# ChenYutongTHU/humannerf

Hardware: AMD Instinct MI355X
Metric: rendered rays/sec (128 samples/ray) at 512x512 (higher is better)
Workload: dtype f32-equivalent: split-f16 hi+lo operands, 3 f16 MFMAs, fp32 accumulate; 1 GPU; BASELINE configs[1]: 512x512 freeview frame, 262144 rays x 128 samples, eval, perturb=0, all 11 outputs of the reference Network.forward; seeded random weights of the default architecture; samples_per_ray=128, ray_chunk=32768, mlp_mode=f16x3, parallelism=frames sharded over 1 GPU(s), no collective

## Files before the change

humannerf_amd/csrc/hnrf_mlp_f16.hip:

```cpp
#include "hnrf_common.h"
#include "hnrf_sincos.h"
#include "hnrf_lds_dma.h"

namespace hnrf {

typedef float f32x16 __attribute__((ext_vector_type(16)));
typedef float f32x2 __attribute__((ext_vector_type(2)));
typedef _Float16 h16x8 __attribute__((ext_vector_type(8)));
typedef _Float16 h16x2 __attribute__((ext_vector_type(2)));

constexpr int RING = 3;
constexpr float LO_SCALE = 2048.0f;
constexpr float LO_INV = 1.0f / 2048.0f;

enum { PE16_NONE = 0, PE16_CANONICAL = 1, PE16_NONRIGID = 2 };

enum { SV_NONE = 0,
       SV_ACT = 1,
       SV_DZ = 2,
       SV_PE = 3,
       SV_ACT_H = 4,
       SV_DZ_H = 5 };
__host__ __device__ constexpr bool sv_fwd(int s) { return s == SV_ACT || s == SV_ACT_H; }
__host__ __device__ constexpr bool sv_bwd(int s) { return s == SV_DZ || s == SV_DZ_H; }
// ... 294 lines not shown
__device__ __forceinline__ void push_pair_bits(uint32_t& acc, h16x2 hh) {
    const unsigned u = __builtin_bit_cast(unsigned, hh);
    unsigned tmp;
    asm("v_pk_min_u16 %1, %2, %3\n\tv_pk_mad_u16 %0, %0, %4, %1" : "+v"(acc), "=&v"(tmp) : "v"(u), "s"(0x00010001u), "s"(0x00020002u));
}

#define HNRF_TILE_EPILOGUE_PAIR(T, I)                                                                                          \
    if constexpr (SAVE == SV_ACT) {                                                                                            \
        float x0, x1;                                                                                                          \
        epi_core<ACT, ULO>(pacc1, pacc2, I, 0u, 0, oh[2 * (T) + ((I) >> 2)], ol[2 * (T) + ((I) >> 2)], x0, x1);                \
        save_pair(*sc, bw, T, I, x0, x1);                                                                                      \
    } else if constexpr (SAVE == SV_ACT_H) {                                                                                   \
        float x0, x1;                                                                                                          \
        const h16x2 hh = epi_core<ACT, ULO>(pacc1, pacc2, I, 0u, 0, oh[2 * (T) + ((I) >> 2)], ol[2 * (T) + ((I) >> 2)], x0, x1); \
        push_pair_bits(bw[(T) >> 1], hh);                                                                                      \
        if ((I) & 1) store_frag_h(rowh, cxh, T, I, oh[2 * (T) + ((I) >> 2)]);                                                  \
    } else if constexpr (SAVE == SV_DZ) {                                                                                      \
        float x0, x1;                                                                                                          \
        epi_core<ACT_MASK_SEL, ULO>(pacc1, pacc2, I, sc->mask[(T) >> 1] >> (16 * ((T) & 1)), 0, oh[2 * (T) + ((I) >> 2)],      \
                                    ol[2 * (T) + ((I) >> 2)], x0, x1);                                                         \
        save_pair_b(*sc, T, I, x0, x1);                                                                                        \
    } else if constexpr (SAVE == SV_DZ_H) {                                                                                    \
        float x0, x1;                                                                                                          \
        const h16x2 hh = epi_core<ACT_MASK_AND, ULO>(pacc1, pacc2, I, sc->mask[(T) >> 1], 8 * ((T) & 1) + (I),                 \
                                                     oh[2 * (T) + ((I) >> 2)], ol[2 * (T) + ((I) >> 2)], x0, x1);              \
        store_pair_h(rowh, cxh, svu, T, I, hh);                                                                                \
    } else if constexpr (SAVE == SV_PE) {                                                                                      \
        sc->fout[16 * (T) + 2 * (I)] = fmaf(pacc2[2 * (I)], LO_INV, pacc1[2 * (I)]);                                           \
        sc->fout[16 * (T) + 2 * (I) + 1] = fmaf(pacc2[2 * (I) + 1], LO_INV, pacc1[2 * (I) + 1]);                               \
    } else                                                                                                                     \
        epi_pair<RELU>(pacc1, I, oh[2 * (T) + ((I) >> 2)], ol[2 * (T) + ((I) >> 2)], p.sat, p.guard);

template <int NT, int TPS, int NKA, int NKB, bool RELU, int SAVE = 0, bool PEND_IN = false, bool DEFER = false,
          int NW = 4, int NB, int NO>
__device__ __forceinline__ void layer16(Pipe& p, int nb1, int nb2, h16x8 (&bh)[NB], h16x8 (&bl)[NB],
                                        h16x8 (&oh)[NO], h16x8 (&ol)[NO], float (&last)[16], SaveCtx* sc = nullptr,
                                        f32x16* pend = nullptr) {
    static_assert(!(PEND_IN || DEFER) || SAVE == SV_NONE, "deferred epilogues exist in the inference form only");
    static_assert(!PEND_IN || NKB >= 2, "a pending tile fills the last two hidden fragments");
    static_assert(NB >= (NKB > 0 ? NKB : 1) && NO >= 2 * NT && NT % TPS == 0, "bad layer shape");
    constexpr int NK = NKA + NKB;
    constexpr int NBLK = 2 * NK;
    constexpr int NS = NT / TPS;
    constexpr int PFK = NK < 4 ? NK : 4;
    static_assert((NBLK * TPS) % NW == 0, "every wave must issue the same number of DMA pieces per slab");
    constexpr bool ULO = !sv_lifted(SAVE);
    constexpr int ACT = RELU ? ACT_RELU : ACT_NONE;
    static_assert(ULO || NT > 1, "the head layers exist in the forward kernels only");
    f32x16 pacc1 = {0.f, 0.f, 0.f, 0.f, 0.f, 0.f, 0.f, 0.f, 0.f, 0.f, 0.f, 0.f, 0.f, 0.f, 0.f, 0.f};
    f32x16 pacc2 = pacc1;
    f32x16 nbias = pacc1;
    uint32_t bw[(NT + 1) / 2];
    _Float16* const rowh = (SAVE == SV_ACT_H || SAVE == SV_DZ_H) ? sc->rowh : nullptr;
    const int cxh = (SAVE == SV_ACT_H || SAVE == SV_DZ_H) ? sc->cx : 0;
    unsigned svu = 0u;
#pragma unroll
    for (int i = 0; i < (NT + 1) / 2; ++i) bw[i] = 0u;
#pragma unroll
    for (int s = 0; s < NS; ++s) {
        const int nissue = (s + 2 < NS) ? NBLK * TPS : (s + 2 == NS ? nb1 : nb2);
        const unsigned slot2 = p.ph == 0 ? 2 : p.ph - 1;
        const int dcnt = nissue / NW;
        const char* dsrc = p.gi + p.wave * dcnt * 1024;
        const unsigned ddst = p.lds_base + p.ring_off + slot2 * p.slab_bytes + p.wave * dcnt * 1024;
        p.gi += nissue * 1024;
#pragma unroll
        for (int tt = 0; tt < TPS; ++tt) {
            const int t = s * TPS + tt;
            const unsigned lane = lane_now();
            unsigned cur = p.lds_base + p.ring_off + p.ph * p.slab_bytes + tt * (NBLK * 1024) + lane * 16;
            unsigned pe = p.lds_base + p.pe_off + p.wave * (PE_STASH / 4) + lane * 16;
            asm volatile("" : "+v"(cur), "+v"(pe));
            f32x16 acc1 = {0.f, 0.f, 0.f, 0.f, 0.f, 0.f, 0.f, 0.f, 0.f, 0.f, 0.f, 0.f, 0.f, 0.f, 0.f, 0.f};
            f32x16 acc2 = acc1;
            if (NT > 1 && sv_has_bias(SAVE)) {
                if (t == 0) {
                    const unsigned bp = p.lds_base + p.bias_off + tt * 128 + (lane >> 5) * 16;
                    const f32x4 b0 = lds_ld4f(bp), b1 = lds_ld4f(bp + 32), b2 = lds_ld4f(bp + 64), b3 = lds_ld4f(bp + 96);
                    acc1 = f32x16{b0.x, b0.y, b0.z, b0.w, b1.x, b1.y, b1.z, b1.w,
                                  b2.x, b2.y, b2.z, b2.w, b3.x, b3.y, b3.z, b3.w};
                } else {
                    acc1 = nbias;
                }
            }
            h16x8 qwh[PFK], qwl[PFK], qxh[PFK], qxl[PFK];
#pragma unroll
            for (int i = 0; i < PFK; ++i) {
                qwh[i] = lds_ld8(cur + (2 * i) * 1024);
                qwl[i] = lds_ld8(cur + (2 * i + 1) * 1024);
                if (i < NKA) {
                    qxh[i] = lds_ld8(pe + (2 * i) * 1024);
                    qxl[i] = lds_ld8(pe + (2 * i + 1) * 1024);
                }
            }
#ifdef HNRF_STAMP
            { const unsigned long long t0 = __builtin_readcyclecounter(); p.sum_b += t0 - p.t_last; p.t_last = t0; }
#endif
            __builtin_amdgcn_sched_barrier(0);
#pragma unroll
            for (int ks = 0; ks < NK; ++ks) {
                const int q = ks % PFK;
                const h16x8 wh = qwh[q], wl = qwl[q];
                h16x8 xh, xl;
                if (ks < NKA) {
                    xh = qxh[q];
                    xl = qxl[q];
                } else {
                    const int ib = ks - NKA < NB ? ks - NKA : 0;
                    xh = bh[ib];
                    xl = bl[ib];
                }
                if (ks + PFK < NK) {
                    qwl[q] = lds_ld8(cur + (2 * (ks + PFK) + 1) * 1024);
                    if (ks + PFK < NKA) qxl[q] = lds_ld8(pe + (2 * (ks + PFK) + 1) * 1024);
                    qwh[q] = lds_ld8(cur + (2 * (ks + PFK)) * 1024);
                    if (ks + PFK < NKA) qxh[q] = lds_ld8(pe + (2 * (ks + PFK)) * 1024);
                }
                acc1 = __builtin_amdgcn_mfma_f32_32x32x16_f16(wh, xh, acc1, 0, 0, 0);
                if (ULO) acc1 = __builtin_amdgcn_mfma_f32_32x32x16_f16(wh, xl, acc1, 0, 0, 0);
                else acc2 = __builtin_amdgcn_mfma_f32_32x32x16_f16(wh, xl, acc2, 0, 0, 0);
                if (ULO) acc1 = __builtin_amdgcn_mfma_f32_32x32x16_f16(wl, xh, acc1, 0, 0, 0);
                else acc2 = __builtin_amdgcn_mfma_f32_32x32x16_f16(wl, xh, acc2, 0, 0, 0);
                if (NT > 1 && sv_has_bias(SAVE) && ks == NK - 1 && t + 1 < NT) {
                    const unsigned bn = p.lds_base + p.bias_off + (tt + 1) * 128 + (lane >> 5) * 16;
                    const f32x4 b0 = lds_ld4f(bn), b1 = lds_ld4f(bn + 32), b2 = lds_ld4f(bn + 64), b3 = lds_ld4f(bn + 96);
                    nbias = f32x16{b0.x, b0.y, b0.z, b0.w, b1.x, b1.y, b1.z, b1.w,
                                   b2.x, b2.y, b2.z, b2.w, b3.x, b3.y, b3.z, b3.w};
                }
                {
                    constexpr int MAXP = (TPS * NK - 1) < 10 ? (TPS * NK - 1) : 10;
                    const int i = tt * NK + ks;
                    if (i >= 0 && i < MAXP) {
                        if (s + 2 < NS) {
                            if (i < NBLK * TPS / NW) dma_run_piece(dsrc, lane * 16, ddst, i);
                        } else if (i < dcnt) {
                            dma_run_piece(dsrc, lane * 16, ddst, i);
                        }
                    }
                }
                if (PEND_IN && t == 0) {
#pragma unroll
                    for (int i = 0; i < 8; ++i)
                        if ((i * (NK - 1)) / 8 == ks) {
                            epi_pair<true>(*pend, i, bh[NKB - 2 + (i >> 2)], bl[NKB - 2 + (i >> 2)], p.sat, p.guard);
                            asm volatile("" : "+v"(bh[NKB - 2 + (i >> 2)]), "+v"(bl[NKB - 2 + (i >> 2)]));
                        }
                }
                if (t > 0) {
#pragma unroll
                    for (int i = 0; i < 8; ++i)
                        if ((i * NK) / 8 == ks) {
                            HNRF_TILE_EPILOGUE_PAIR(t - 1, i)
                            if constexpr (SAVE != SV_PE)
                                asm volatile("" : "+v"(oh[2 * (t - 1) + (i >> 2)]), "+v"(ol[2 * (t - 1) + (i >> 2)]));
                        }
                }
                __builtin_amdgcn_sched_group_barrier(0x008, 1, 0);
                __builtin_amdgcn_sched_group_barrier(0x002, 6, 0);
                __builtin_amdgcn_sched_group_barrier(0x008, 1, 0);
                __builtin_amdgcn_sched_group_barrier(0x100, 2, 0);
                __builtin_amdgcn_sched_group_barrier(0x002, 5, 0);
                __builtin_amdgcn_sched_group_barrier(0x008, 1, 0);
                __builtin_amdgcn_sched_group_barrier(0x002, 8, 0);
                __builtin_amdgcn_sched_barrier(0);
            }
#ifdef HNRF_STAMP
            { const unsigned long long t1 = __builtin_readcyclecounter(); p.sum_k += t1 - p.t_last; p.t_last = t1; }
#endif
            pacc1 = acc1;
            pacc2 = acc2;
        }
        const int n_st = (sv_fwd(SAVE) || sv_bwd(SAVE)) ? 4 * (s == 0 ? TPS - 1 : TPS) : 0;
        tile_sync(nissue / NW + n_st);
        p.ph = p.ph == RING - 1 ? 0 : p.ph + 1;
        p.bias_off += TPS * 128;
    }
    if (NT == 1) {
#pragma unroll
        for (int r = 0; r < 16; ++r) last[r] = pacc1[r];
    } else if (DEFER) {
        *pend = pacc1;
    } else {
#pragma unroll
        for (int i = 0; i < 8; ++i) {
            HNRF_TILE_EPILOGUE_PAIR(NT - 1, i)
        }
        if constexpr (sv_fwd(SAVE)) {
#pragma unroll
            for (int i = 0; i < (NT + 1) / 2; ++i) sc->bits[i] = bw[i];
        }
    }
}

#undef HNRF_TILE_EPILOGUE_PAIR

template <int NT, int TPS, int NKA, int NKB, bool RELU, int NB, int NO>
__device__ __forceinline__ void layer16x2(Pipe& p, unsigned stash_per_wave, int nb1, int nb2,
                                          const h16x8 (&bh)[2][NB], const h16x8 (&bl)[2][NB], h16x8 (&oh)[2][NO],
                                          h16x8 (&ol)[2][NO], float (&last)[2][16]) {
    static_assert(NB >= (NKB > 0 ? NKB : 1) && NO >= 2 * NT && NT % TPS == 0, "bad layer shape");
    constexpr int NK = NKA + NKB;
    constexpr int NBLK = 2 * NK;
    constexpr int NS = NT / TPS;
    constexpr int PFK = NK < 4 ? NK : 4;
    static_assert((NBLK * TPS) % 4 == 0, "every wave must issue the same number of DMA pieces per slab");
    const f32x16 zero = {0.f, 0.f, 0.f, 0.f, 0.f, 0.f, 0.f, 0.f, 0.f, 0.f, 0.f, 0.f, 0.f, 0.f, 0.f, 0.f};
    f32x16 pacc[2] = {zero, zero};
#pragma unroll
    for (int s = 0; s < NS; ++s) {
        const int nissue = (s + 2 < NS) ? NBLK * TPS : (s + 2 == NS ? nb1 : nb2);
        const unsigned slot2 = p.ph == 0 ? 2 : p.ph - 1;
        const int dcnt = nissue / 4;
        const char* dsrc = p.gi + p.wave * dcnt * 1024;
        const unsigned ddst = p.lds_base + p.ring_off + slot2 * p.slab_bytes + p.wave * dcnt * 1024;
        p.gi += nissue * 1024;
#pragma unroll
        for (int tt = 0; tt < TPS; ++tt) {
            const int t = s * TPS + tt;
            const unsigned lane = lane_now();
            unsigned cur = p.lds_base + p.ring_off + p.ph * p.slab_bytes + tt * (NBLK * 1024) + lane * 16;
            unsigned pe = p.lds_base + p.pe_off + p.wave * stash_per_wave + lane * 16;
            asm volatile("" : "+v"(cur), "+v"(pe));
            f32x16 acc[2] = {zero, zero};
            if (NT > 1) {
                const unsigned bp = p.lds_base + p.bias_off + tt * 128 + (lane >> 5) * 16;
                const f32x4 b0 = lds_ld4f(bp), b1 = lds_ld4f(bp + 32), b2 = lds_ld4f(bp + 64), b3 = lds_ld4f(bp + 96);
                acc[0] = f32x16{b0.x, b0.y, b0.z, b0.w, b1.x, b1.y, b1.z, b1.w,
                                 b2.x, b2.y, b2.z, b2.w, b3.x, b3.y, b3.z, b3.w};
                acc[1] = acc[0];
            }
            h16x8 qwh[PFK], qwl[PFK], qxh[2][PFK], qxl[2][PFK];
#pragma unroll
            for (int i = 0; i < PFK; ++i) {
                qwh[i] = lds_ld8(cur + (2 * i) * 1024);
                qwl[i] = lds_ld8(cur + (2 * i + 1) * 1024);
                if (i < NKA) {
#pragma unroll
                    for (int g = 0; g < 2; ++g) {
                        qxh[g][i] = lds_ld8(pe + g * (stash_per_wave / 2) + (2 * i) * 1024);
                        qxl[g][i] = lds_ld8(pe + g * (stash_per_wave / 2) + (2 * i + 1) * 1024);
                    }
                }
            }
            __builtin_amdgcn_sched_barrier(0);
#pragma unroll
            for (int ks = 0; ks < NK; ++ks) {
                const int q = ks % PFK;
                const h16x8 wh = qwh[q], wl = qwl[q];
                h16x8 xh[2], xl[2];
#pragma unroll
                for (int g = 0; g < 2; ++g) {
                    if (ks < NKA) {
                        xh[g] = qxh[g][q];
                        xl[g] = qxl[g][q];
                    } else {
                        const int ib = ks - NKA < NB ? ks - NKA : 0;
                        xh[g] = bh[g][ib];
                        xl[g] = bl[g][ib];
                    }
                }
                if (ks + PFK < NK) {
                    qwl[q] = lds_ld8(cur + (2 * (ks + PFK) + 1) * 1024);
                    if (ks + PFK < NKA) {
#pragma unroll
                        for (int g = 1; g >= 0; --g) qxl[g][q] = lds_ld8(pe + g * (stash_per_wave / 2) + (2 * (ks + PFK) + 1) * 1024);
                    }
                    qwh[q] = lds_ld8(cur + (2 * (ks + PFK)) * 1024);
                    if (ks + PFK < NKA) {
#pragma unroll
                        for (int g = 1; g >= 0; --g) qxh[g][q] = lds_ld8(pe + g * (stash_per_wave / 2) + (2 * (ks + PFK)) * 1024);
                    }
                }
#pragma unroll
                for (int g = 0; g < 2; ++g) {
                    acc[g] = __builtin_amdgcn_mfma_f32_32x32x16_f16(wh, xh[g], acc[g], 0, 0, 0);
                    acc[g] = __builtin_amdgcn_mfma_f32_32x32x16_f16(wh, xl[g], acc[g], 0, 0, 0);
                    acc[g] = __builtin_amdgcn_mfma_f32_32x32x16_f16(wl, xh[g], acc[g], 0, 0, 0);
                }
                {
                    constexpr int MAXP = (TPS * NK - 1) < 10 ? (TPS * NK - 1) : 10;
                    const int i = tt * NK + ks;
                    if (i >= 0 && i < MAXP) {
                        if (s + 2 < NS) {
                            if (i < NBLK * TPS / 4) dma_run_piece(dsrc, lane * 16, ddst, i);
                        } else if (i < dcnt) {
                            dma_run_piece(dsrc, lane * 16, ddst, i);
                        }
                    }
                }
                if (t > 0) {
#pragma unroll
                    for (int j = 0; j < 16; ++j)
                        if ((j * NK) / 16 == ks) {
                            const int g = j >> 3, i = j & 7;
                            epi_pair<RELU>(pacc[g], i, oh[g][2 * (t - 1) + (i >> 2)], ol[g][2 * (t - 1) + (i >> 2)], p.sat, p.guard);
                            asm volatile("" : "+v"(oh[g][2 * (t - 1) + (i >> 2)]), "+v"(ol[g][2 * (t - 1) + (i >> 2)]));
                        }
                }
                __builtin_amdgcn_sched_group_barrier(0x008, 1, 0);
                __builtin_amdgcn_sched_group_barrier(0x002, 6, 0);
                __builtin_amdgcn_sched_group_barrier(0x008, 1, 0);
                __builtin_amdgcn_sched_group_barrier(0x100, 2, 0);
                __builtin_amdgcn_sched_group_barrier(0x002, 5, 0);
                __builtin_amdgcn_sched_group_barrier(0x008, 1, 0);
                __builtin_amdgcn_sched_group_barrier(0x100, 2, 0);
                __builtin_amdgcn_sched_group_barrier(0x002, 5, 0);
                __builtin_amdgcn_sched_group_barrier(0x008, 1, 0);
                __builtin_amdgcn_sched_group_barrier(0x002, 6, 0);
                __builtin_amdgcn_sched_group_barrier(0x008, 1, 0);
                __builtin_amdgcn_sched_group_barrier(0x100, 2, 0);
                __builtin_amdgcn_sched_group_barrier(0x002, 5, 0);
                __builtin_amdgcn_sched_group_barrier(0x008, 1, 0);
                __builtin_amdgcn_sched_group_barrier(0x002, 8, 0);
                __builtin_amdgcn_sched_barrier(0);
            }
#pragma unroll
            for (int g = 0; g < 2; ++g) pacc[g] = acc[g];
        }
        tile_sync(nissue / 4);
        p.ph = p.ph == RING - 1 ? 0 : p.ph + 1;
        p.bias_off += TPS * 128;
    }
#pragma unroll
    for (int g = 0; g < 2; ++g) {
        if (NT == 1) {
#pragma unroll
            for (int r = 0; r < 16; ++r) last[g][r] = pacc[g][r];
        } else {
#pragma unroll
            for (int i = 0; i < 8; ++i)
                epi_pair<RELU>(pacc[g], i, oh[g][2 * (NT - 1) + (i >> 2)], ol[g][2 * (NT - 1) + (i >> 2)], p.sat, p.guard);
        }
    }
}

__device__ __forceinline__ Pipe pipe_start(const char* packed, int64_t bias_img_off, int bias_bytes, int slab_bytes,
                                           int nb0, int nb1, char* smem, int stash_bytes = PE_STASH, int nw = 4) {
    Pipe p;
    p.wave = __builtin_amdgcn_readfirstlane(threadIdx.x >> 6);
    p.lds_base = __builtin_amdgcn_readfirstlane((unsigned)(size_t)(lds_char*)smem);
    p.pe_off = bias_bytes;
    p.ring_off = bias_bytes + stash_bytes;
    p.slab_bytes = slab_bytes;
    p.ph = 0;
    p.bias_off = 0;
    p.sat = 0ull;
    p.guard = false;
#ifdef HNRF_STAMP
    p.t_last = __builtin_readcyclecounter();
    p.sum_k = p.sum_b = 0;
#endif
    slab_issue(packed + bias_img_off, p.lds_base, bias_bytes / 1024, p.wave, nw);
    slab_issue(packed, p.lds_base + p.ring_off, nb0, p.wave, nw);
    slab_issue(packed + nb0 * 1024, p.lds_base + p.ring_off + slab_bytes, nb1, p.wave, nw);
    p.gi = packed + (nb0 + nb1) * 1024;
    return p;
}

template <bool ULO = false>
__device__ __forceinline__ void stash_pe(const Pipe& p, int ks, const float (&v)[8]) {
    h16x8 hi, lo;
    split8<ULO>(v, hi, lo);
    const unsigned pe = p.lds_base + p.pe_off + p.wave * (PE_STASH / 4) + lane_now() * 16;
    lds_st8(pe + (2 * ks) * 1024, hi);
    lds_st8(pe + (2 * ks + 1) * 1024, lo);
}

// ... 75 lines not shown
    layer16<1, 1, 0, 16, false, 0, DF, false>(p, 0, 0, hA_h, hA_l, dh, dl, last, nullptr, &pend);
    const float* ob = reinterpret_cast<const float*>(packed + CNL16_BIAS + CNL16_BIAS_LDS);
    if constexpr (HEADS) {
        if (slot < P) {
#pragma unroll
            for (int q = 0; q < 4; ++q) {
                const int g = 2 * q + h;
                if (g < n_heads) {
                    const float hs = h ? ob[32 + 2 * q + 1] : ob[32 + 2 * q];
                    const float* bg = ob + 4 * g;
                    raw[(int64_t)g * plane + sample] = make_float4(fmaf(last[4 * q], hs, bg[0]), fmaf(last[4 * q + 1], hs, bg[1]),
                                                                   fmaf(last[4 * q + 2], hs, bg[2]), fmaf(last[4 * q + 3], hs, bg[3]));
                }
            }
        }
    } else {
        const float hs = ob[8];
        if (h == 0 && slot < P)
            raw[sample] = make_float4(fmaf(last[0], hs, ob[0]), fmaf(last[1], hs, ob[1]), fmaf(last[2], hs, ob[2]), fmaf(last[3], hs, ob[3]));
    }
    if constexpr (SAVE == SV_NONE && GUARD) raise_f16_range(packed, CNL16_STATUS, p.sat);
#ifdef HNRF_STAMP
    if (threadIdx.x == 0 && blockIdx.x < 4096) {
        const unsigned long long te = __builtin_readcyclecounter();
        unsigned long long* dbg = (unsigned long long*)(const_cast<char*>(packed) + CNL16_BYTES);
        dbg[blockIdx.x * 4 + 0] = p.sum_k; dbg[blockIdx.x * 4 + 1] = p.sum_b + (te - p.t_last);
    }
#endif
}

constexpr int NR16W8_SLAB = 24 * 1024;
constexpr int NR16W8_STASH = 64 * 1024;

template <int SAVE, int NW = 4>
__global__ __launch_bounds__(64 * NW) void nonrigid_f16x3_kernel(const float* __restrict__ x_skel,
                                                             const float* __restrict__ hann_w,
                                                             const char* __restrict__ packed, int64_t P,
                                                             float* __restrict__ xyz, float* __restrict__ offsets,
                                                             const int* __restrict__ idx,
                                                             const int* __restrict__ count,
                                                             float* __restrict__ pe_out, float* __restrict__ acts,
                                                             uint32_t* __restrict__ relu_bits) {
    extern __shared__ __attribute__((aligned(16))) char smem[];
    if (idx != nullptr) {
        P = *count;
        if ((int64_t)blockIdx.x * (32 * NW) >= P) return;
    }
    static_assert(NW == 4 || NW == 8, "waves per workgroup");
    constexpr bool W8 = NW == 8;
    Pipe p = W8 ? pipe_start(packed, NR16_BIAS, NR16_BIAS_LDS, NR16W8_SLAB, 2 * NR16_NB_L0, 2 * NR16_NB_L0, smem, NR16W8_STASH, 8)
                : pipe_start(packed, NR16_BIAS, NR16_BIAS_LDS, NR16_SLAB, 4 * NR16_NB_L0, 2 * NR16_NB_MID, smem);
    const int lane = threadIdx.x & 63, h = lane >> 5;
    const int64_t slot = ((int64_t)blockIdx.x * NW + p.wave) * 32 + (lane & 31);
    const int64_t sclamp = slot < P ? slot : P - 1;
    const int64_t sidx = idx ? (int64_t)idx[sclamp] : sclamp;
    const int64_t sample = slot < P ? sidx : P;

    const float x[3] = {x_skel[sidx * 3 + 0], x_skel[sidx * 3 + 1], x_skel[sidx * 3 + 2]};
    float pev[32];
    pe_sincos_shared<6>(x, h, pev);
#pragma unroll
    for (int a = 0; a < 18; ++a) pev[a] *= hann_w[a / 3];
#pragma unroll
    for (int a = 18; a < 32; ++a) pev[a] = 0.f;
#pragma unroll
    for (int ks = 0; ks < 4; ++ks) {
        const float v[8] = {pev[8 * ks], pev[8 * ks + 1], pev[8 * ks + 2], pev[8 * ks + 3],
                            pev[8 * ks + 4], pev[8 * ks + 5], pev[8 * ks + 6], pev[8 * ks + 7]};
        stash_pe<true>(p, ks, v);
    }
    SaveCtx sc;
    if constexpr (SAVE) {
        sc.row = acts + sidx * 128 + 4 * h;
        sc.rowh = reinterpret_cast<_Float16*>(acts) + (slot >> 5) * (128 * 32) + h * 128;
        sc.cx = (lane & 31) ^ (4 * h);
        sc.bits = relu_bits + sidx * 4 + 2 * h;
        if constexpr (SAVE == SV_ACT_H) {
            _Float16* ph = reinterpret_cast<_Float16*>(pe_out) + sidx * 64;
#pragma unroll
            for (int a = 0; a < 18; ++a) ph[pe_col16(PE16_NONRIGID, a, h)] = (_Float16)pev[a];
#pragma unroll
            for (int a = 18; a < 32; ++a) ph[36 + 2 * (a - 18) + h] = (_Float16)0.f;
        } else {
#pragma unroll
            for (int a = 0; a < 18; ++a) pe_out[sidx * 36 + pe_col16(PE16_NONRIGID, a, h)] = pev[a];
        }
    }
    const int64_t act_stride = P * 128, bit_stride = P * 4;
    const int64_t acth_stride = (int64_t)gridDim.x * (32 * NW) * 128;
    tile_sync(0);

    h16x8 hA_h[8], hA_l[8], hB_h[8], hB_l[8];
    float last[16];
    h16x8 dh[2], dl[2];
    if constexpr (W8) {
        constexpr int MID = NR16_NB_MID, L4B = NR16_NB_L4;
#define HNRF_NEXT_LAYER if constexpr (SAVE) { sc.row += act_stride; sc.rowh += acth_stride; sc.bits += bit_stride; }
        layer16<4, 2, 4, 0, true, SAVE, false, false, 8>(p, MID, MID, hB_h, hB_l, hA_h, hA_l, last, &sc);
        HNRF_NEXT_LAYER
        layer16<4, 1, 0, 8, true, SAVE, false, false, 8>(p, MID, MID, hA_h, hA_l, hB_h, hB_l, last, &sc);
        HNRF_NEXT_LAYER
        layer16<4, 1, 0, 8, true, SAVE, false, false, 8>(p, MID, MID, hB_h, hB_l, hA_h, hA_l, last, &sc);
        HNRF_NEXT_LAYER
        layer16<4, 1, 0, 8, true, SAVE, false, false, 8>(p, L4B, L4B, hA_h, hA_l, hB_h, hB_l, last, &sc);
        HNRF_NEXT_LAYER
        layer16<4, 1, 4, 8, true, SAVE, false, false, 8>(p, MID, MID, hB_h, hB_l, hA_h, hA_l, last, &sc);
        HNRF_NEXT_LAYER
        layer16<4, 1, 0, 8, true, SAVE, false, false, 8>(p, MID, 0, hA_h, hA_l, hB_h, hB_l, last, &sc);
#undef HNRF_NEXT_LAYER
        layer16<1, 1, 0, 8, false, 0, false, false, 8>(p, 0, 0, hB_h, hB_l, dh, dl, last);
    } else {
    layer16<4, 4, 4, 0, true, SAVE>(p, 0 , 2 * NR16_NB_MID, hB_h, hB_l, hA_h, hA_l, last, &sc);
    if constexpr (SAVE) { sc.row += act_stride; sc.rowh += acth_stride; sc.bits += bit_stride; }
    layer16<4, 2, 0, 8, true, SAVE>(p, 2 * NR16_NB_MID, 2 * NR16_NB_MID, hA_h, hA_l, hB_h, hB_l, last, &sc);
    if constexpr (SAVE) { sc.row += act_stride; sc.rowh += acth_stride; sc.bits += bit_stride; }
    layer16<4, 2, 0, 8, true, SAVE>(p, 2 * NR16_NB_MID, 2 * NR16_NB_MID, hB_h, hB_l, hA_h, hA_l, last, &sc);
    if constexpr (SAVE) { sc.row += act_stride; sc.rowh += acth_stride; sc.bits += bit_stride; }
    layer16<4, 2, 0, 8, true, SAVE>(p, NR16_NB_L4, NR16_NB_L4, hA_h, hA_l, hB_h, hB_l, last, &sc);
    if constexpr (SAVE) { sc.row += act_stride; sc.rowh += acth_stride; sc.bits += bit_stride; }
    layer16<4, 1, 4, 8, true, SAVE>(p, 2 * NR16_NB_MID, 2 * NR16_NB_MID, hB_h, hB_l, hA_h, hA_l, last, &sc);
    if constexpr (SAVE) { sc.row += act_stride; sc.rowh += acth_stride; sc.bits += bit_stride; }
    layer16<4, 2, 0, 8, true, SAVE>(p, NR16_NB_MID, 0, hA_h, hA_l, hB_h, hB_l, last, &sc);
    layer16<1, 1, 0, 8, false, 0>(p, 0, 0, hB_h, hB_l, dh, dl, last);
    }
    const float* ob = reinterpret_cast<const float*>(packed + NR16_BIAS + NR16_BIAS_LDS);
    const float hs = ob[8];
    if (h == 0 && slot < P) {
        const float o0 = fmaf(last[0], hs, ob[0]), o1 = fmaf(last[1], hs, ob[1]), o2 = fmaf(last[2], hs, ob[2]);
        xyz[sample * 3 + 0] = x[0] + o0;
        xyz[sample * 3 + 1] = x[1] + o1;
        xyz[sample * 3 + 2] = x[2] + o2;
        if (offsets) {
            offsets[sample * 3 + 0] = o0;
            offsets[sample * 3 + 1] = o1;
            offsets[sample * 3 + 2] = o2;
        }
    }
}

constexpr int NR16X2_SLAB = 24 * 1024;
constexpr int NR16X2_STASH = 64 * 1024;

template <bool GUARD>
__global__ __launch_bounds__(256) void nonrigid_f16x3_x2_kernel(const float* __restrict__ x_skel,
                                                                const float* __restrict__ hann_w,
                                                                const char* __restrict__ packed, int64_t P,
                                                                float* __restrict__ xyz, float* __restrict__ offsets,
                                                                const int* __restrict__ idx,
                                                                const int* __restrict__ count) {
    extern __shared__ __attribute__((aligned(16))) char smem[];
    if (idx != nullptr) {
        P = *count;
        if ((int64_t)blockIdx.x * 256 >= P) return;
    }
    Pipe p = pipe_start(packed, NR16_BIAS, NR16_BIAS_LDS, NR16X2_SLAB, 2 * NR16_NB_L0, 2 * NR16_NB_L0, smem,
                        NR16X2_STASH);
    p.guard = GUARD;
    constexpr unsigned SPW = NR16X2_STASH / 4;
    const int lane = threadIdx.x & 63, h = lane >> 5;
    int64_t sidx[2];
    bool live[2];
    float x[2][3];
#pragma unroll
    for (int g = 0; g < 2; ++g) {
        const int64_t slot = ((int64_t)blockIdx.x * 4 + p.wave) * 64 + g * 32 + (lane & 31);
        const int64_t sclamp = slot < P ? slot : P - 1;
        sidx[g] = idx ? (int64_t)idx[sclamp] : sclamp;
        live[g] = slot < P;
#pragma unroll
        for (int a = 0; a < 3; ++a) x[g][a] = x_skel[sidx[g] * 3 + a];
    }
#pragma unroll
    for (int g = 0; g < 2; ++g) {
        float pev[32];
        pe_sincos_shared<6>(x[g], h, pev);
#pragma unroll
        for (int a = 0; a < 18; ++a) pev[a] *= hann_w[a / 3];
#pragma unroll
        for (int a = 18; a < 32; ++a) pev[a] = 0.f;
        const unsigned pe = p.lds_base + p.pe_off + p.wave * SPW + g * (SPW / 2) + lane_now() * 16;
#pragma unroll
        for (int ks = 0; ks < 4; ++ks) {
            const float v[8] = {pev[8 * ks], pev[8 * ks + 1], pev[8 * ks + 2], pev[8 * ks + 3],
                                pev[8 * ks + 4], pev[8 * ks + 5], pev[8 * ks + 6], pev[8 * ks + 7]};
            h16x8 hi, lo;
            split8<true>(v, hi, lo);
            lds_st8(pe + (2 * ks) * 1024, hi);
            lds_st8(pe + (2 * ks + 1) * 1024, lo);
        }
    }
    tile_sync(0);

    h16x8 hA_h[2][8], hA_l[2][8], hB_h[2][8], hB_l[2][8];
    float last[2][16];
    constexpr int MID = NR16_NB_MID, L4B = NR16_NB_L4;
    layer16x2<4, 2, 4, 0, true>(p, SPW, MID, MID, hB_h, hB_l, hA_h, hA_l, last);
    layer16x2<4, 1, 0, 8, true>(p, SPW, MID, MID, hA_h, hA_l, hB_h, hB_l, last);
    layer16x2<4, 1, 0, 8, true>(p, SPW, MID, MID, hB_h, hB_l, hA_h, hA_l, last);
    layer16x2<4, 1, 0, 8, true>(p, SPW, L4B, L4B, hA_h, hA_l, hB_h, hB_l, last);
    layer16x2<4, 1, 4, 8, true>(p, SPW, MID, MID, hB_h, hB_l, hA_h, hA_l, last);
    layer16x2<4, 1, 0, 8, true>(p, SPW, MID, 0, hA_h, hA_l, hB_h, hB_l, last);
    h16x8 dh[2][2], dl[2][2];
    layer16x2<1, 1, 0, 8, false>(p, SPW, 0, 0, hB_h, hB_l, dh, dl, last);
    const float* ob = reinterpret_cast<const float*>(packed + NR16_BIAS + NR16_BIAS_LDS);
    const float hs = ob[8];
#pragma unroll
    for (int g = 0; g < 2; ++g) {
        if (h == 0 && live[g]) {
            const float o0 = fmaf(last[g][0], hs, ob[0]), o1 = fmaf(last[g][1], hs, ob[1]), o2 = fmaf(last[g][2], hs, ob[2]);
            xyz[sidx[g] * 3 + 0] = x[g][0] + o0;
            xyz[sidx[g] * 3 + 1] = x[g][1] + o1;
            xyz[sidx[g] * 3 + 2] = x[g][2] + o2;
            if (offsets) {
                offsets[sidx[g] * 3 + 0] = o0;
                offsets[sidx[g] * 3 + 1] = o1;
                offsets[sidx[g] * 3 + 2] = o2;
            }
        }
    }
    if constexpr (GUARD) raise_f16_range(packed, NR16_STATUS, p.sat);
}

struct PackBwd16 {
    const float* W;
    int n_out, n_in;
    int NT, NK;
    int row_kind;
    int col0;
    int head;
    int64_t off;
    const float* amax;
};

struct LayerSet {
    const float* w[9];
    int n[9];
};
__global__ __launch_bounds__(256) void layer_amax_kernel(LayerSet ls, float* __restrict__ out) {
    __shared__ float red[256];
    const float* W = ls.w[blockIdx.x];
    const int n = ls.n[blockIdx.x];
    float m = 0.f;
    for (int e = blockIdx.y * 256 + threadIdx.x; e < n; e += 256 * gridDim.y) m = fmaxf(m, fabsf(W[e]));
    red[threadIdx.x] = m;
    __syncthreads();
    for (int st = 128; st >= 1; st >>= 1) {
        if ((int)threadIdx.x < st) red[threadIdx.x] = fmaxf(red[threadIdx.x], red[threadIdx.x + st]);
        __syncthreads();
    }
    if (threadIdx.x == 0) atomicMax(reinterpret_cast<unsigned int*>(out) + blockIdx.x, __float_as_uint(red[0]));
}

struct PackBwdSet16 {
// ... 378 lines not shown
    return launch_lds<canonical_f16x3_kernel<SV_NONE, false, true>>(what, grid, dim3(256), lds, st, xyz, (const char*)packed, P,
                                                                    (float4*)raw, idx, count, nullptr, nullptr, nullptr,
                                                                    n_heads);
}

int canonical16_fwd_train(const float* xyz, const void* packed, int64_t P, float* raw, float* pe_out, float* acts,
                          uint32_t* relu_bits, int half, hipStream_t st) {
    constexpr int lds = CNL16_BIAS_LDS + PE_STASH + RING * CNL16_SLAB;
    const dim3 grid((unsigned)((P + 127) / 128));
    const char* what = "hnrf_canonical_fwd_train (f16x3)";
    if (half)
        return launch_lds<canonical_f16x3_kernel<SV_ACT_H>>(what, grid, dim3(256), lds, st, xyz, (const char*)packed, P,
                                                            (float4*)raw, nullptr, nullptr, pe_out, acts, relu_bits, 1);
    return launch_lds<canonical_f16x3_kernel<SV_ACT>>(what, grid, dim3(256), lds, st, xyz, (const char*)packed, P, (float4*)raw,
                                                      nullptr, nullptr, pe_out, acts, relu_bits, 1);
}

int canonical16_heads_fwd_train(const float* xyz, const void* packed, int64_t P, int n_heads, float* raw, float* pe_out,
                                float* acts, uint32_t* relu_bits, int half, hipStream_t st) {
    constexpr int lds = CNL16_BIAS_LDS + PE_STASH + RING * CNL16_SLAB;
    const dim3 grid((unsigned)((P + 127) / 128));
    const char* what = "hnrf_canonical_heads_fwd_train (f16x3)";
    if (half)
        return launch_lds<canonical_f16x3_kernel<SV_ACT_H, false, true>>(what, grid, dim3(256), lds, st, xyz, (const char*)packed,
                                                                         P, (float4*)raw, nullptr, nullptr, pe_out, acts,
                                                                         relu_bits, n_heads);
    return launch_lds<canonical_f16x3_kernel<SV_ACT, false, true>>(what, grid, dim3(256), lds, st, xyz, (const char*)packed, P,
                                                                   (float4*)raw, nullptr, nullptr, pe_out, acts, relu_bits,
                                                                   n_heads);
}

int nonrigid16_fwd(const float* x_skel, const float* hann_w, const void* packed, int64_t P, float* xyz,
                   float* offsets, const int* idx, const int* count, bool guard, hipStream_t st) {
    constexpr int lds2 = NR16_BIAS_LDS + NR16X2_STASH + RING * NR16X2_SLAB;
    const dim3 grid((unsigned)((P + 255) / 256));
    const char* what = "hnrf_nonrigid_fwd (f16x3)";
    if (guard)
        return launch_lds<nonrigid_f16x3_x2_kernel<true>>(what, grid, dim3(256), lds2, st, x_skel, hann_w, (const char*)packed, P,
                                                          xyz, offsets, idx, count);
    return launch_lds<nonrigid_f16x3_x2_kernel<false>>(what, grid, dim3(256), lds2, st, x_skel, hann_w, (const char*)packed, P,
                                                       xyz, offsets, idx, count);
}

int nonrigid16_fwd_train(const float* x_skel, const float* hann_w, const void* packed, int64_t P, float* xyz,
                         float* offsets, float* pe_out, float* acts, uint32_t* relu_bits, int half, hipStream_t st) {
    constexpr int lds = NR16_BIAS_LDS + PE_STASH + RING * NR16_SLAB;
    const dim3 grid((unsigned)((P + 127) / 128));
    const char* what = "hnrf_nonrigid_fwd_train (f16x3)";
    if (half && P % 256 == 0) {
        constexpr int lds8 = NR16_BIAS_LDS + NR16W8_STASH + RING * NR16W8_SLAB;
        return launch_lds<nonrigid_f16x3_kernel<SV_ACT_H, 8>>(what, dim3((unsigned)(P / 256)), dim3(512), lds8, st, x_skel, hann_w,
                                                              (const char*)packed, P, xyz, offsets, nullptr, nullptr, pe_out,
                                                              acts, relu_bits);
    }
    if (half)
        return launch_lds<nonrigid_f16x3_kernel<SV_ACT_H>>(what, grid, dim3(256), lds, st, x_skel, hann_w, (const char*)packed, P,
                                                           xyz, offsets, nullptr, nullptr, pe_out, acts, relu_bits);
    return launch_lds<nonrigid_f16x3_kernel<SV_ACT>>(what, grid, dim3(256), lds, st, x_skel, hann_w, (const char*)packed, P, xyz,
                                                     offsets, nullptr, nullptr, pe_out, acts, relu_bits);
}

size_t canonical16_bwd_bytes() { return (size_t)CB16_BYTES + 256; }

static int launch_layer_amax(const float* const* w, const int* n, int count, float* out, hipStream_t st) {
    LayerSet ls;
    for (int i = 0; i < 9; ++i) { ls.w[i] = i < count ? w[i] : nullptr; ls.n[i] = i < count ? n[i] : 0; }
    if (hipMemsetAsync(out, 0, 256, st) != hipSuccess) {
        set_error("hnrf pack (layer maxima): memset failed");
        return HNRF_E_LAUNCH;
    }
    hipLaunchKernelGGL(layer_amax_kernel, dim3(count, 16), dim3(256), 0, st, ls, out);
    return check_launch("hnrf pack (layer maxima)");
}

// ... 110 lines not shown
```

Baseline: 4.968 million rays/s.

## Route nonrigid inference through 8-wave kernel with deferred epilogues and mid-slab sync

Removes the dedicated two-group nonrigid inference kernel. Inference now runs through the 8-wave nonrigid kernel (512 threads, one 32-row tile per wave) with deferred epilogues. A new MIDSYNC mode moves the ring barrier to the middle of each slab's MFMA loop and issues the next slab's DMA pieces after it, so the barrier is hidden behind compute instead of sitting at the slab's end. The trade is more waves per block and a different barrier placement, which may change register pressure and occupancy compared with the old register-blocked two-group design.

New measurement: 4.989 million rays/s (median of 6 runs). Within noise of the previous version (+0.4%).

```diff
diff --git a/humannerf_amd/csrc/hnrf_mlp_f16.hip b/humannerf_amd/csrc/hnrf_mlp_f16.hip
--- a/humannerf_amd/csrc/hnrf_mlp_f16.hip
+++ b/humannerf_amd/csrc/hnrf_mlp_f16.hip
@@ -350,7 +350,7 @@
         epi_pair<RELU>(pacc1, I, oh[2 * (T) + ((I) >> 2)], ol[2 * (T) + ((I) >> 2)], p.sat, p.guard);
 
 template <int NT, int TPS, int NKA, int NKB, bool RELU, int SAVE = 0, bool PEND_IN = false, bool DEFER = false,
-          int NW = 4, int NB, int NO>
+          int NW = 4, bool MIDSYNC = false, int NB, int NO>
 __device__ __forceinline__ void layer16(Pipe& p, int nb1, int nb2, h16x8 (&bh)[NB], h16x8 (&bl)[NB],
                                         h16x8 (&oh)[NO], h16x8 (&ol)[NO], float (&last)[16], SaveCtx* sc = nullptr,
                                         f32x16* pend = nullptr) {
@@ -365,6 +365,9 @@
     constexpr bool ULO = !sv_lifted(SAVE);
     constexpr int ACT = RELU ? ACT_RELU : ACT_NONE;
     static_assert(ULO || NT > 1, "the head layers exist in the forward kernels only");
+    static_assert(!MIDSYNC || SAVE == SV_NONE, "the activation stores of the training forms are counted at the slab's end");
+    constexpr int MS = TPS * NK / 2;
+    static_assert(!MIDSYNC || 24 / NW <= TPS * NK - MS, "a slab's pieces (at most 24 blocks) are issued behind the meeting");
     f32x16 pacc1 = {0.f, 0.f, 0.f, 0.f, 0.f, 0.f, 0.f, 0.f, 0.f, 0.f, 0.f, 0.f, 0.f, 0.f, 0.f, 0.f};
     f32x16 pacc2 = pacc1;
     f32x16 nbias = pacc1;
@@ -417,6 +420,10 @@
             __builtin_amdgcn_sched_barrier(0);
 #pragma unroll
             for (int ks = 0; ks < NK; ++ks) {
+                if (MIDSYNC && tt * NK + ks == MS) {
+                    tile_sync(0);
+                    __builtin_amdgcn_sched_barrier(0);
+                }
                 const int q = ks % PFK;
                 const h16x8 wh = qwh[q], wl = qwl[q];
                 h16x8 xh, xl;
@@ -447,7 +454,7 @@
                 }
                 {
                     constexpr int MAXP = (TPS * NK - 1) < 10 ? (TPS * NK - 1) : 10;
-                    const int i = tt * NK + ks;
+                    const int i = tt * NK + ks - (MIDSYNC ? MS : 0);
                     if (i >= 0 && i < MAXP) {
                         if (s + 2 < NS) {
                             if (i < NBLK * TPS / NW) dma_run_piece(dsrc, lane * 16, ddst, i);
@@ -489,7 +496,7 @@
             pacc2 = acc2;
         }
         const int n_st = (sv_fwd(SAVE) || sv_bwd(SAVE)) ? 4 * (s == 0 ? TPS - 1 : TPS) : 0;
-        tile_sync(nissue / NW + n_st);
+        if constexpr (!MIDSYNC) tile_sync(nissue / NW + n_st);
         p.ph = p.ph == RING - 1 ? 0 : p.ph + 1;
         p.bias_off += TPS * 128;
     }
@@ -511,146 +518,6 @@
 }
 
 #undef HNRF_TILE_EPILOGUE_PAIR
-
-template <int NT, int TPS, int NKA, int NKB, bool RELU, int NB, int NO>
-__device__ __forceinline__ void layer16x2(Pipe& p, unsigned stash_per_wave, int nb1, int nb2,
-                                          const h16x8 (&bh)[2][NB], const h16x8 (&bl)[2][NB], h16x8 (&oh)[2][NO],
-                                          h16x8 (&ol)[2][NO], float (&last)[2][16]) {
-    static_assert(NB >= (NKB > 0 ? NKB : 1) && NO >= 2 * NT && NT % TPS == 0, "bad layer shape");
-    constexpr int NK = NKA + NKB;
-    constexpr int NBLK = 2 * NK;
-    constexpr int NS = NT / TPS;
-    constexpr int PFK = NK < 4 ? NK : 4;
-    static_assert((NBLK * TPS) % 4 == 0, "every wave must issue the same number of DMA pieces per slab");
-    const f32x16 zero = {0.f, 0.f, 0.f, 0.f, 0.f, 0.f, 0.f, 0.f, 0.f, 0.f, 0.f, 0.f, 0.f, 0.f, 0.f, 0.f};
-    f32x16 pacc[2] = {zero, zero};
-#pragma unroll
-    for (int s = 0; s < NS; ++s) {
-        const int nissue = (s + 2 < NS) ? NBLK * TPS : (s + 2 == NS ? nb1 : nb2);
-        const unsigned slot2 = p.ph == 0 ? 2 : p.ph - 1;
-        const int dcnt = nissue / 4;
-        const char* dsrc = p.gi + p.wave * dcnt * 1024;
-        const unsigned ddst = p.lds_base + p.ring_off + slot2 * p.slab_bytes + p.wave * dcnt * 1024;
-        p.gi += nissue * 1024;
-#pragma unroll
-        for (int tt = 0; tt < TPS; ++tt) {
-            const int t = s * TPS + tt;
-            const unsigned lane = lane_now();
-            unsigned cur = p.lds_base + p.ring_off + p.ph * p.slab_bytes + tt * (NBLK * 1024) + lane * 16;
-            unsigned pe = p.lds_base + p.pe_off + p.wave * stash_per_wave + lane * 16;
-            asm volatile("" : "+v"(cur), "+v"(pe));
-            f32x16 acc[2] = {zero, zero};
-            if (NT > 1) {
-                const unsigned bp = p.lds_base + p.bias_off + tt * 128 + (lane >> 5) * 16;
-                const f32x4 b0 = lds_ld4f(bp), b1 = lds_ld4f(bp + 32), b2 = lds_ld4f(bp + 64), b3 = lds_ld4f(bp + 96);
-                acc[0] = f32x16{b0.x, b0.y, b0.z, b0.w, b1.x, b1.y, b1.z, b1.w,
-                                 b2.x, b2.y, b2.z, b2.w, b3.x, b3.y, b3.z, b3.w};
-                acc[1] = acc[0];
-            }
-            h16x8 qwh[PFK], qwl[PFK], qxh[2][PFK], qxl[2][PFK];
-#pragma unroll
-            for (int i = 0; i < PFK; ++i) {
-                qwh[i] = lds_ld8(cur + (2 * i) * 1024);
-                qwl[i] = lds_ld8(cur + (2 * i + 1) * 1024);
-                if (i < NKA) {
-#pragma unroll
-                    for (int g = 0; g < 2; ++g) {
-                        qxh[g][i] = lds_ld8(pe + g * (stash_per_wave / 2) + (2 * i) * 1024);
-                        qxl[g][i] = lds_ld8(pe + g * (stash_per_wave / 2) + (2 * i + 1) * 1024);
-                    }
-                }
-            }
-            __builtin_amdgcn_sched_barrier(0);
-#pragma unroll
-            for (int ks = 0; ks < NK; ++ks) {
-                const int q = ks % PFK;
-                const h16x8 wh = qwh[q], wl = qwl[q];
-                h16x8 xh[2], xl[2];
-#pragma unroll
-                for (int g = 0; g < 2; ++g) {
-                    if (ks < NKA) {
-                        xh[g] = qxh[g][q];
-                        xl[g] = qxl[g][q];
-                    } else {
-                        const int ib = ks - NKA < NB ? ks - NKA : 0;
-                        xh[g] = bh[g][ib];
-                        xl[g] = bl[g][ib];
-                    }
-                }
-                if (ks + PFK < NK) {
-                    qwl[q] = lds_ld8(cur + (2 * (ks + PFK) + 1) * 1024);
-                    if (ks + PFK < NKA) {
-#pragma unroll
-                        for (int g = 1; g >= 0; --g) qxl[g][q] = lds_ld8(pe + g * (stash_per_wave / 2) + (2 * (ks + PFK) + 1) * 1024);
-                    }
-                    qwh[q] = lds_ld8(cur + (2 * (ks + PFK)) * 1024);
-                    if (ks + PFK < NKA) {
-#pragma unroll
-                        for (int g = 1; g >= 0; --g) qxh[g][q] = lds_ld8(pe + g * (stash_per_wave / 2) + (2 * (ks + PFK)) * 1024);
-                    }
-                }
-#pragma unroll
-                for (int g = 0; g < 2; ++g) {
-                    acc[g] = __builtin_amdgcn_mfma_f32_32x32x16_f16(wh, xh[g], acc[g], 0, 0, 0);
-                    acc[g] = __builtin_amdgcn_mfma_f32_32x32x16_f16(wh, xl[g], acc[g], 0, 0, 0);
-                    acc[g] = __builtin_amdgcn_mfma_f32_32x32x16_f16(wl, xh[g], acc[g], 0, 0, 0);
-                }
-                {
-                    constexpr int MAXP = (TPS * NK - 1) < 10 ? (TPS * NK - 1) : 10;
-                    const int i = tt * NK + ks;
-                    if (i >= 0 && i < MAXP) {
-                        if (s + 2 < NS) {
-                            if (i < NBLK * TPS / 4) dma_run_piece(dsrc, lane * 16, ddst, i);
-                        } else if (i < dcnt) {
-                            dma_run_piece(dsrc, lane * 16, ddst, i);
-                        }
-                    }
-                }
-                if (t > 0) {
-#pragma unroll
-                    for (int j = 0; j < 16; ++j)
-                        if ((j * NK) / 16 == ks) {
-                            const int g = j >> 3, i = j & 7;
-                            epi_pair<RELU>(pacc[g], i, oh[g][2 * (t - 1) + (i >> 2)], ol[g][2 * (t - 1) + (i >> 2)], p.sat, p.guard);
-                            asm volatile("" : "+v"(oh[g][2 * (t - 1) + (i >> 2)]), "+v"(ol[g][2 * (t - 1) + (i >> 2)]));
-                        }
-                }
-                __builtin_amdgcn_sched_group_barrier(0x008, 1, 0);
-                __builtin_amdgcn_sched_group_barrier(0x002, 6, 0);
-                __builtin_amdgcn_sched_group_barrier(0x008, 1, 0);
-                __builtin_amdgcn_sched_group_barrier(0x100, 2, 0);
-                __builtin_amdgcn_sched_group_barrier(0x002, 5, 0);
-                __builtin_amdgcn_sched_group_barrier(0x008, 1, 0);
-                __builtin_amdgcn_sched_group_barrier(0x100, 2, 0);
-                __builtin_amdgcn_sched_group_barrier(0x002, 5, 0);
-                __builtin_amdgcn_sched_group_barrier(0x008, 1, 0);
-                __builtin_amdgcn_sched_group_barrier(0x002, 6, 0);
-                __builtin_amdgcn_sched_group_barrier(0x008, 1, 0);
-                __builtin_amdgcn_sched_group_barrier(0x100, 2, 0);
-                __builtin_amdgcn_sched_group_barrier(0x002, 5, 0);
-                __builtin_amdgcn_sched_group_barrier(0x008, 1, 0);
-                __builtin_amdgcn_sched_group_barrier(0x002, 8, 0);
-                __builtin_amdgcn_sched_barrier(0);
-            }
-#pragma unroll
-            for (int g = 0; g < 2; ++g) pacc[g] = acc[g];
-        }
-        tile_sync(nissue / 4);
-        p.ph = p.ph == RING - 1 ? 0 : p.ph + 1;
-        p.bias_off += TPS * 128;
-    }
-#pragma unroll
-    for (int g = 0; g < 2; ++g) {
-        if (NT == 1) {
-#pragma unroll
-            for (int r = 0; r < 16; ++r) last[g][r] = pacc[g][r];
-        } else {
-#pragma unroll
-            for (int i = 0; i < 8; ++i)
-                epi_pair<RELU>(pacc[g], i, oh[g][2 * (NT - 1) + (i >> 2)], ol[g][2 * (NT - 1) + (i >> 2)], p.sat, p.guard);
-        }
-    }
-}
 
 __device__ __forceinline__ Pipe pipe_start(const char* packed, int64_t bias_img_off, int bias_bytes, int slab_bytes,
                                            int nb0, int nb1, char* smem, int stash_bytes = PE_STASH, int nw = 4) {
@@ -792,7 +659,7 @@
 constexpr int NR16W8_SLAB = 24 * 1024;
 constexpr int NR16W8_STASH = 64 * 1024;
 
-template <int SAVE, int NW = 4>
+template <int SAVE, int NW = 4, bool GUARD = false>
 __global__ __launch_bounds__(64 * NW) void nonrigid_f16x3_kernel(const float* __restrict__ x_skel,
                                                              const float* __restrict__ hann_w,
                                                              const char* __restrict__ packed, int64_t P,
@@ -810,6 +677,7 @@
     constexpr bool W8 = NW == 8;
     Pipe p = W8 ? pipe_start(packed, NR16_BIAS, NR16_BIAS_LDS, NR16W8_SLAB, 2 * NR16_NB_L0, 2 * NR16_NB_L0, smem, NR16W8_STASH, 8)
                 : pipe_start(packed, NR16_BIAS, NR16_BIAS_LDS, NR16_SLAB, 4 * NR16_NB_L0, 2 * NR16_NB_MID, smem);
+    p.guard = GUARD && SAVE == SV_NONE;
     const int lane = threadIdx.x & 63, h = lane >> 5;
     const int64_t slot = ((int64_t)blockIdx.x * NW + p.wave) * 32 + (lane & 31);
     const int64_t sclamp = slot < P ? slot : P - 1;
@@ -849,26 +717,31 @@
     const int64_t act_stride = P * 128, bit_stride = P * 4;
     const int64_t acth_stride = (int64_t)gridDim.x * (32 * NW) * 128;
     tile_sync(0);
+#ifdef HNRF_STAMP
+    const unsigned long long t_pro = __builtin_readcyclecounter() - p.t_last;
+#endif
 
     h16x8 hA_h[8], hA_l[8], hB_h[8], hB_l[8];
     float last[16];
     h16x8 dh[2], dl[2];
     if constexpr (W8) {
         constexpr int MID = NR16_NB_MID, L4B = NR16_NB_L4;
+        constexpr bool INF = SAVE == SV_NONE;
+        f32x16 pend;
 #define HNRF_NEXT_LAYER if constexpr (SAVE) { sc.row += act_stride; sc.rowh += acth_stride; sc.bits += bit_stride; }
-        layer16<4, 2, 4, 0, true, SAVE, false, false, 8>(p, MID, MID, hB_h, hB_l, hA_h, hA_l, last, &sc);
+        layer16<4, 2, 4, 0, true, SAVE, false, INF, 8, INF>(p, MID, MID, hB_h, hB_l, hA_h, hA_l, last, &sc, &pend);
         HNRF_NEXT_LAYER
-        layer16<4, 1, 0, 8, true, SAVE, false, false, 8>(p, MID, MID, hA_h, hA_l, hB_h, hB_l, last, &sc);
+        layer16<4, 1, 0, 8, true, SAVE, INF, INF, 8, INF>(p, MID, MID, hA_h, hA_l, hB_h, hB_l, last, &sc, &pend);
         HNRF_NEXT_LAYER
-        layer16<4, 1, 0, 8, true, SAVE, false, false, 8>(p, MID, MID, hB_h, hB_l, hA_h, hA_l, last, &sc);
+        layer16<4, 1, 0, 8, true, SAVE, INF, INF, 8, INF>(p, MID, MID, hB_h, hB_l, hA_h, hA_l, last, &sc, &pend);
         HNRF_NEXT_LAYER
-        layer16<4, 1, 0, 8, true, SAVE, false, false, 8>(p, L4B, L4B, hA_h, hA_l, hB_h, hB_l, last, &sc);
+        layer16<4, 1, 0, 8, true, SAVE, INF, INF, 8, INF>(p, L4B, L4B, hA_h, hA_l, hB_h, hB_l, last, &sc, &pend);
         HNRF_NEXT_LAYER
-        layer16<4, 1, 4, 8, true, SAVE, false, false, 8>(p, MID, MID, hB_h, hB_l, hA_h, hA_l, last, &sc);
+        layer16<4, 1, 4, 8, true, SAVE, INF, INF, 8, INF>(p, MID, MID, hB_h, hB_l, hA_h, hA_l, last, &sc, &pend);
         HNRF_NEXT_LAYER
-        layer16<4, 1, 0, 8, true, SAVE, false, false, 8>(p, MID, 0, hA_h, hA_l, hB_h, hB_l, last, &sc);
+        layer16<4, 1, 0, 8, true, SAVE, INF, INF, 8, INF>(p, MID, 0, hA_h, hA_l, hB_h, hB_l, last, &sc, &pend);
 #undef HNRF_NEXT_LAYER
-        layer16<1, 1, 0, 8, false, 0, false, false, 8>(p, 0, 0, hB_h, hB_l, dh, dl, last);
+        layer16<1, 1, 0, 8, false, 0, INF, false, 8, INF>(p, 0, 0, hB_h, hB_l, dh, dl, last, nullptr, &pend);
     } else {
     layer16<4, 4, 4, 0, true, SAVE>(p, 0 , 2 * NR16_NB_MID, hB_h, hB_l, hA_h, hA_l, last, &sc);
     if constexpr (SAVE) { sc.row += act_stride; sc.rowh += acth_stride; sc.bits += bit_stride; }
@@ -896,89 +769,14 @@
             offsets[sample * 3 + 2] = o2;
         }
     }
-}
-
-constexpr int NR16X2_SLAB = 24 * 1024;
-constexpr int NR16X2_STASH = 64 * 1024;
-
-template <bool GUARD>
-__global__ __launch_bounds__(256) void nonrigid_f16x3_x2_kernel(const float* __restrict__ x_skel,
-                                                                const float* __restrict__ hann_w,
-                                                                const char* __restrict__ packed, int64_t P,
-                                                                float* __restrict__ xyz, float* __restrict__ offsets,
-                                                                const int* __restrict__ idx,
-                                                                const int* __restrict__ count) {
-    extern __shared__ __attribute__((aligned(16))) char smem[];
-    if (idx != nullptr) {
-        P = *count;
-        if ((int64_t)blockIdx.x * 256 >= P) return;
-    }
-    Pipe p = pipe_start(packed, NR16_BIAS, NR16_BIAS_LDS, NR16X2_SLAB, 2 * NR16_NB_L0, 2 * NR16_NB_L0, smem,
-                        NR16X2_STASH);
-    p.guard = GUARD;
-    constexpr unsigned SPW = NR16X2_STASH / 4;
-    const int lane = threadIdx.x & 63, h = lane >> 5;
-    int64_t sidx[2];
-    bool live[2];
-    float x[2][3];
-#pragma unroll
-    for (int g = 0; g < 2; ++g) {
-        const int64_t slot = ((int64_t)blockIdx.x * 4 + p.wave) * 64 + g * 32 + (lane & 31);
-        const int64_t sclamp = slot < P ? slot : P - 1;
-        sidx[g] = idx ? (int64_t)idx[sclamp] : sclamp;
-        live[g] = slot < P;
-#pragma unroll
-        for (int a = 0; a < 3; ++a) x[g][a] = x_skel[sidx[g] * 3 + a];
-    }
-#pragma unroll
-    for (int g = 0; g < 2; ++g) {
-        float pev[32];
-        pe_sincos_shared<6>(x[g], h, pev);
-#pragma unroll
-        for (int a = 0; a < 18; ++a) pev[a] *= hann_w[a / 3];
-#pragma unroll
-        for (int a = 18; a < 32; ++a) pev[a] = 0.f;
-        const unsigned pe = p.lds_base + p.pe_off + p.wave * SPW + g * (SPW / 2) + lane_now() * 16;
-#pragma unroll
-        for (int ks = 0; ks < 4; ++ks) {
-            const float v[8] = {pev[8 * ks], pev[8 * ks + 1], pev[8 * ks + 2], pev[8 * ks + 3],
-                                pev[8 * ks + 4], pev[8 * ks + 5], pev[8 * ks + 6], pev[8 * ks + 7]};
-            h16x8 hi, lo;
-            split8<true>(v, hi, lo);
-            lds_st8(pe + (2 * ks) * 1024, hi);
-            lds_st8(pe + (2 * ks + 1) * 1024, lo);
-        }
-    }
-    tile_sync(0);
-
-    h16x8 hA_h[2][8], hA_l[2][8], hB_h[2][8], hB_l[2][8];
-    float last[2][16];
-    constexpr int MID = NR16_NB_MID, L4B = NR16_NB_L4;
-    layer16x2<4, 2, 4, 0, true>(p, SPW, MID, MID, hB_h, hB_l, hA_h, hA_l, last);
-    layer16x2<4, 1, 0, 8, true>(p, SPW, MID, MID, hA_h, hA_l, hB_h, hB_l, last);
-    layer16x2<4, 1, 0, 8, true>(p, SPW, MID, MID, hB_h, hB_l, hA_h, hA_l, last);
-    layer16x2<4, 1, 0, 8, true>(p, SPW, L4B, L4B, hA_h, hA_l, hB_h, hB_l, last);
-    layer16x2<4, 1, 4, 8, true>(p, SPW, MID, MID, hB_h, hB_l, hA_h, hA_l, last);
-    layer16x2<4, 1, 0, 8, true>(p, SPW, MID, 0, hA_h, hA_l, hB_h, hB_l, last);
-    h16x8 dh[2][2], dl[2][2];
-    layer16x2<1, 1, 0, 8, false>(p, SPW, 0, 0, hB_h, hB_l, dh, dl, last);
-    const float* ob = reinterpret_cast<const float*>(packed + NR16_BIAS + NR16_BIAS_LDS);
-    const float hs = ob[8];
-#pragma unroll
-    for (int g = 0; g < 2; ++g) {
-        if (h == 0 && live[g]) {
-            const float o0 = fmaf(last[g][0], hs, ob[0]), o1 = fmaf(last[g][1], hs, ob[1]), o2 = fmaf(last[g][2], hs, ob[2]);
-            xyz[sidx[g] * 3 + 0] = x[g][0] + o0;
-            xyz[sidx[g] * 3 + 1] = x[g][1] + o1;
-            xyz[sidx[g] * 3 + 2] = x[g][2] + o2;
-            if (offsets) {
-                offsets[sidx[g] * 3 + 0] = o0;
-                offsets[sidx[g] * 3 + 1] = o1;
-                offsets[sidx[g] * 3 + 2] = o2;
-            }
-        }
-    }
-    if constexpr (GUARD) raise_f16_range(packed, NR16_STATUS, p.sat);
+    if constexpr (SAVE == SV_NONE && GUARD) raise_f16_range(packed, NR16_STATUS, p.sat);
+#ifdef HNRF_STAMP
+    if ((threadIdx.x & 63) == 0 && (p.wave & 3) == 0 && blockIdx.x < 4096) {
+        const unsigned long long te = __builtin_readcyclecounter();
+        unsigned long long* dbg = (unsigned long long*)(const_cast<char*>(packed) + NR16_BYTES) + (blockIdx.x * 2 + (p.wave >> 2)) * 4;
+        dbg[0] = p.sum_k; dbg[1] = p.sum_b + (te - p.t_last); dbg[2] = t_pro; dbg[3] = te - p.t_last;
+    }
+#endif
 }
 
 struct PackBwd16 {
@@ -1423,14 +1221,15 @@
 
 int nonrigid16_fwd(const float* x_skel, const float* hann_w, const void* packed, int64_t P, float* xyz,
                    float* offsets, const int* idx, const int* count, bool guard, hipStream_t st) {
-    constexpr int lds2 = NR16_BIAS_LDS + NR16X2_STASH + RING * NR16X2_SLAB;
+    constexpr int lds8 = NR16_BIAS_LDS + NR16W8_STASH + RING * NR16W8_SLAB;
     const dim3 grid((unsigned)((P + 255) / 256));
     const char* what = "hnrf_nonrigid_fwd (f16x3)";
     if (guard)
-        return launch_lds<nonrigid_f16x3_x2_kernel<true>>(what, grid, dim3(256), lds2, st, x_skel, hann_w, (const char*)packed, P,
-                                                          xyz, offsets, idx, count);
-    return launch_lds<nonrigid_f16x3_x2_kernel<false>>(what, grid, dim3(256), lds2, st, x_skel, hann_w, (const char*)packed, P,
-                                                       xyz, offsets, idx, count);
+        return launch_lds<nonrigid_f16x3_kernel<SV_NONE, 8, true>>(what, grid, dim3(512), lds8, st, x_skel, hann_w,
+                                                                   (const char*)packed, P, xyz, offsets, idx, count, nullptr,
+                                                                   nullptr, nullptr);
+    return launch_lds<nonrigid_f16x3_kernel<SV_NONE, 8>>(what, grid, dim3(512), lds8, st, x_skel, hann_w, (const char*)packed, P,
+                                                         xyz, offsets, idx, count, nullptr, nullptr, nullptr);
 }
 
 int nonrigid16_fwd_train(const float* x_skel, const float* hann_w, const void* packed, int64_t P, float* xyz,
```
